# jacketsj/expANN

Hardware: AMD Instinct MI355X
Metric: queries/sec at recall@10=1.0 (exact brute force), 1Mxd128 fp32, k=10 (higher is better)
Workload: dtype f32; 1 GPU; brute_force_engine L2 N=1000000 d=128 fp32, 10000 batched queries, k=10 (BASELINE configs[1]); n=1000000, d=128, m=10000, k=10, metric=l2, launch=one process, one GPU, devices_visible=1, comm_ranks=0

## Files before the change

expann_amd/csrc/expann_hip.hip:

```cpp
#include "../../include/expann_hip.h"

#include <hip/hip_runtime.h>

#include <algorithm>
#include <cmath>
#include <cstdio>
#include <cstdlib>
#include <cstring>
#include <memory>
#include <mutex>
#include <string>
#include <vector>

#include "host_common.hpp"
#include "scan_f32.hpp"
#include "scan_gemm_bf16.hpp"
#include "scan_gemm_f16.hpp"
#include "scan_gemm_f16k.hpp"
#include "scan_gemm_f16x.hpp"
#include "scan_gemm_f16y.hpp"
#include "scan_gemm_f16kx.hpp"
#include "scan_gemm_f16kl.hpp"
#include "scan_direct_f16.hpp"
#include "scan_gemm_i8.hpp"
// ... 608 lines not shown
#define GEMM_I8(D, MODE, MN) {D, MODE, scan_gemm_i8_kernel<D, MODE>, row_self_i8_kernel<D, MODE>, \
	query_theta_i8_kernel<D, MODE>, "scan_gemm_i8<" #D "," MN ">"}
const GemmI8Variant kGemmI8[] = {
    GEMM_I8(128, kU8L2, "U8L2"), GEMM_I8(128, kI8L2, "I8L2"), GEMM_I8(128, kI8IP, "I8IP"),
    GEMM_I8(256, kU8L2, "U8L2"), GEMM_I8(256, kI8L2, "I8L2"), GEMM_I8(256, kI8IP, "I8IP"),
    GEMM_I8(768, kU8L2, "U8L2"), GEMM_I8(768, kI8L2, "I8L2"), GEMM_I8(768, kI8IP, "I8IP")};
#undef GEMM_I8

const GemmI8Variant* pick_gemm_i8(const expann_index* h, size_t m) {
	if (h->opt_scan_kernel == 1 || h->dtype == EXPANN_DTYPE_F32)
		return nullptr;
	if (h->opt_scan_kernel == 0 && (m < 96 || h->n < 4096))
		return nullptr;
	for (const auto& v : kGemmI8)
		if (v.d == h->dim && v.mode == h->int_mode)
			return &v;
	return nullptr;
}

int ensure_bias_i8(expann_index* h, const GemmI8Variant* gv, hipStream_t st) {
	if (h->d_bias_i || h->int_mode == kI8IP)
		return EXPANN_OK;
	HIP_TRY(h, hipMalloc(&h->d_bias_i, sizeof(int) * h->n));
	const uint32_t blocks = (uint32_t)((h->n + kRowsPerGroup - 1) / kRowsPerGroup);
	hipLaunchKernelGGL(gv->self, dim3(blocks), dim3(kBlock), 0, st, (const void*)h->d_base,
	                   (uint32_t)h->n, h->d_bias_i);
	HIP_TRY(h, hipGetLastError());
	return EXPANN_OK;
}

uint32_t select_longest_list(double expect, uint32_t spec_j) {
	return spec_j ? (uint32_t)(expect * (1.0 + 4.5 / std::sqrt((double)spec_j))) : 2u * (uint32_t)expect;
}
void launch_select_wave(SelectParams& sel, size_t m, uint32_t cap, hipStream_t st, uint32_t longest) {
	sel.wave_done = 0;
	hipLaunchKernelGGL((select_wave_kernel<8, 4>), dim3((uint32_t)((m + 3) / 4)), dim3(256), 0, st, sel,
	                   (uint32_t)m);
	sel.wave_done = 512;
	if (longest <= 512)
		return;
	if (cap > 512) {
		hipLaunchKernelGGL((select_wave_kernel<16, 2>), dim3((uint32_t)((m + 1) / 2)), dim3(128), 0, st, sel, (uint32_t)m);
		sel.wave_done = 1024;
	}
	if (cap > 1024 && longest > 1024) {
		hipLaunchKernelGGL((select_wave_kernel<32, 1>), dim3((uint32_t)m), dim3(64), 0, st, sel, (uint32_t)m);
		sel.wave_done = 2048;
	}
}

int ensure_hit_logs(expann_index* h, uint32_t grid, int waves, size_t m, uint32_t cap, uint32_t n_chunks,
                    uint32_t n_qtiles, uint32_t xcd_map, hipStream_t st, uint4** log, uint32_t** log_cnt,
                    uint32_t* log_cap_out) {
	const uint32_t n_logs = grid * (uint32_t)waves;
	const uint32_t log_cap = std::max<uint32_t>(
	    4096, pow2ceil((uint32_t)std::min<size_t>(4 * ((m * (size_t)cap + n_logs - 1) / n_logs), 1u << 20)));
	const size_t need = (size_t)n_logs * log_cap * 16;
	if (need > h->log_bytes || n_logs > h->log_cnt_n) {
		HIP_TRY(h, hipStreamSynchronize(st));
		h->d_log.reset();
		h->d_log_cnt.reset();
		h->log_bytes = h->log_cnt_n = 0;
		HIP_TRY(h, hipMalloc(&h->d_log, need));
		HIP_TRY(h, hipMalloc(&h->d_log_cnt, sizeof(uint32_t) * n_logs));
		h->log_bytes = need;
		h->log_cnt_n = n_logs;
	}
	*log = h->d_log.as<uint4>();
	*log_cnt = h->d_log_cnt;
	*log_cap_out = log_cap;
	h->pending_scatter.n_logs = n_logs;
	h->pending_scatter.log_cap = log_cap;
	h->pending_scatter.cap = cap;
	h->pending_scatter.n_chunks = n_chunks;
	h->pending_scatter.n_qtiles = n_qtiles;
	h->pending_scatter.xcd_map = xcd_map;
	h->pending_scatter.m = (uint32_t)m;
	h->pending_scatter.theta = nullptr;
	h->pending_scatter.key_mul = 0.0f;
	h->pending_scatter.i_mode = 0;
	return EXPANN_OK;
}

void launch_gather_logs(expann_index* h, hipStream_t st) {
	if (!h->pending_scatter.n_logs)
		return;
	const auto ps = h->pending_scatter;
	h->pending_scatter.n_logs = 0;
	const uint32_t want = std::max<uint32_t>(1, (1024 + ps.n_qtiles * 4 - 1) / (ps.n_qtiles * 4));
	const uint32_t cpb = std::max<uint32_t>(1, (ps.n_chunks + want - 1) / want);
	const uint32_t n_groups = (ps.n_chunks + cpb - 1) / cpb;
	GatherLogParams gp{h->d_log.as<const uint4>(), h->d_log_cnt.as<const uint32_t>(), ps.log_cap, ps.n_chunks,
	                   ps.n_qtiles, ps.xcd_map, ps.m, n_groups, cpb, h->d_cnt, h->d_cand, ps.cap, ps.theta, ps.key_mul,
	                   ps.i_thp, ps.i_bias, ps.i_qself, ps.i_mode, ps.i_rw};
	hipLaunchKernelGGL(gather_logs_kernel, dim3(ps.n_qtiles * 4 * n_groups), dim3(kBlock), 0, st, gp);
}

bool defer_flags(expann_index* h, hipStream_t st, int attempt) {
	if (!h->opt_async || h->host_call || attempt != 0 || h->strict_u8 || h->async_pending >= kAsyncRing)
		return false;
	if (hipMemcpyAsync(h->h_flag_ring + 8 * h->async_pending, h->d_overflow,
	                   sizeof(uint32_t) * 4 + sizeof(unsigned long long), hipMemcpyDeviceToHost, st) != hipSuccess)
		return false;
	h->h_flag_ring[8 * h->async_pending + 6] = 0;
	h->h_flag_ring[8 * h->async_pending + 7] = h->dtype == EXPANN_DTYPE_U8 ? 1u : 0u;
	h->async_pending++;
	h->async_stream = st;
	h->prof.deferred_searches++;
	return true;
}

uint32_t pick_row_chunks(uint32_t n_tiles, uint32_t n_qtiles, uint32_t slots, double overhead, uint32_t min_tiles,
                         uint32_t g_limit, long tol_pct, uint32_t* xcd) {
	const uint32_t gmax = std::max<uint32_t>(1, n_tiles / min_tiles);
	uint32_t chunks = 1, g8 = 0;
	double best = 1e300, best8 = 1e300;
	for (uint32_t g = 1; g <= std::min<uint32_t>(gmax, g_limit); ++g) {
		const uint32_t steps = (n_tiles + g - 1) / g;
		const uint64_t rounds = ((uint64_t)g * n_qtiles + slots - 1) / slots;
		const double cost = (double)rounds * (steps + overhead);
		if (cost < best * 0.999) {
			best = cost;
			chunks = g;
		}
		if (xcd && g % 8 == 0 && cost < best8 * 0.999 && (n_tiles + steps - 1) / steps == g) {
			best8 = cost;
			g8 = g;
		}
// ... 355 lines not shown
		fp.cand_cnt = h->d_cnt;
		fp.cand = h->d_cand;
		fp.cap = cap;
		const GemmI8qVariant* gs = gq;
		const uint32_t scan_slots = gs->scan_w ? (uint32_t)gs->wg_per_cu_w * (uint32_t)cus : wg_slots;
		uint32_t fchunks = pick_row_chunks(nt, nqt, scan_slots, 4.0, 8, 2048, h->opt_xcd_tolerance,
		                                   (h->opt_debug & 1024) ? nullptr : &fp.xcd_map);
		fp.tiles_per_block = (nt + fchunks - 1) / fchunks;
		fchunks = (nt + fp.tiles_per_block - 1) / fp.tiles_per_block;
		GemmI8wParams wp{};
		if (gs->scan_w) {
			wp.q = fp;
			rc = ensure_hit_logs(h, fchunks * nqt, 4, m, cap, fchunks, nqt, fp.xcd_map, st, &wp.log, &wp.log_cnt,
			                     &wp.log_cap);
			if (rc != EXPANN_OK)
				return rc;
			wp.lost = h->d_overflow;
			h->pending_scatter.i_thp = fp.thp;
			h->pending_scatter.i_bias = fp.bias;
			h->pending_scatter.i_qself = fp.qself;
			h->pending_scatter.i_mode = fp.bias ? 1 : 2;
		}
		const bool timed = h->profiling && h->ev_used < kEventPairs;
		if (timed)
			HIP_TRY(h, hipEventRecord(h->ev[h->ev_used][0], st));
		if (gs->scan_w)
			hipLaunchKernelGGL(gs->scan_w, dim3(fchunks * nqt), dim3((uint32_t)gs->threads_w), gs->lds_w, st, wp);
		else
			hipLaunchKernelGGL(gs->scan, dim3(fchunks * nqt), dim3((uint32_t)gs->threads), gs->lds, st, fp);
		if (timed) {
			HIP_TRY(h, hipEventRecord(h->ev[h->ev_used][1], st));
			h->ev_used++;
		}
		launch_gather_logs(h, st);
		if (timed || !h->profiling) {
			h->prof.scan_launches++;
			h->prof.scan_rows += h->n;
			h->prof.scan_query_tiles += nqt;
			h->prof.query_tile = kF16TQ;
			h->prof.levels = 2;
			std::snprintf(h->prof.scan_kernel, sizeof(h->prof.scan_kernel), "%s", gs->name);
		}
		HIP_TRY(h, hipGetLastError());
		mark("scan");
		SelectParams sel{};
		sel.cand = h->d_cand;
		sel.cand_cnt = h->d_cnt;
		sel.cap = cap;
		sel.k = (uint32_t)k;
		sel.id_offset = h->id_offset;
		sel.out_ids = d_ids;
		sel.out_dists = d_dists;
		sel.dim = (uint32_t)h->dim;
		sel.overflow = h->d_overflow;
		if (h->profiling)
			hipLaunchKernelGGL(sum_u32_kernel, dim3(1), dim3(1024), 0, st, sel.cand_cnt, (uint32_t)m,
			                   h->d_total);
		launch_select_wave(sel, m, cap, st, select_longest_list(1.2 * (double)k * sample_frac_for(h, k), 0));
		mark("select_wave");
		hipLaunchKernelGGL(select_topk_kernel, dim3((uint32_t)m), dim3(kBlock), sizeof(uint64_t) * cap + 16,
		                   st, sel);
		HIP_TRY(h, hipGetLastError());
		if (defer_flags(h, st, attempt)) {
			h->h_flag_ring[8 * (h->async_pending - 1) + 6] = 0;
			return EXPANN_OK;
		}
		HIP_TRY(h, hipMemcpyAsync(h->h_flags, h->d_overflow, sizeof(uint32_t) * 4 + sizeof(unsigned long long),
		                          hipMemcpyDeviceToHost, st));
		HIP_TRY(h, hipStreamSynchronize(st));
		unsigned long long tot;
		std::memcpy(&tot, h->h_flags + 4, sizeof(tot));
		h->prof.candidates = tot;
		if (h->strict_u8 && (h->h_flags[1] != 0 || h->h_flags[3] != 0))
			return kStrictReject;
		if (h->dtype == EXPANN_DTYPE_U8 && h->h_flags[1] != 0)
			return h->fail(EXPANN_ERR_UNSUPPORTED,
			               std::to_string(h->h_flags[1]) +
			                   " query values outside [0,255]: the uint8 metric "
			                   "(dist2_compressed) is only defined for 8-bit valued queries");
		if (h->h_flags[0] == 0)
			return EXPANN_OK;
		h->prof.retries++;
		if (cap >= kMaxCap || attempt >= 2)
			return kRetryGeneric;
		cap = std::min(cap * 4, kMaxCap);
	}
}

int search_pass(expann_index* h, const void* d_queries, size_t m, size_t k, uint64_t* d_ids,
                float* d_dists, hipStream_t st);
}
extern "C" int expann_create(int dim, int dtype, int metric, int device, expann_index** out);
extern "C" int expann_set_base_device(expann_index* h, const void* d_rows, size_t n, uint64_t id_offset);
extern "C" int expann_set_profiling(expann_index* h, int enable);
// ... 718 lines not shown
		gp.bias = h->d_bias_i;
		gp.n_rows = (uint32_t)h->n;
		const uint32_t n_tiles = (uint32_t)((h->n + tb - 1) / tb);
		gp.n_tiles_sel = last ? n_tiles
		                      : std::min(n_tiles, (L.n_groups_sel * kRowsPerGroup + tb - 1) / tb);
		gp.tile_stride = std::max<uint32_t>(1, n_tiles / gp.n_tiles_sel);
		gp.n_qtiles = (uint32_t)((m + kGemmI8TQ - 1) / kGemmI8TQ);
		gp.queries = d_queries;
		gp.theta = h->d_theta.as<const int>();
		gp.qself = h->d_qself;
		gp.m = (uint32_t)m;
		gp.cand_cnt = h->d_cnt;
		gp.cand = h->d_cand;
		gp.cap = cap;
		uint32_t gchunks = pick_row_chunks(gp.n_tiles_sel, gp.n_qtiles, (uint32_t)cus, 2.0, 4, 4096, 0, nullptr);
		gp.tiles_per_block = (gp.n_tiles_sel + gchunks - 1) / gchunks;
		gchunks = (gp.n_tiles_sel + gp.tiles_per_block - 1) / gp.tiles_per_block;
		if (timed)
			HIP_TRY(h, hipEventRecord(h->ev[h->ev_used][0], st));
		hipLaunchKernelGGL(gvi->scan, dim3(gchunks * gp.n_qtiles), dim3(kGemmThreads),
		                   2 * tb * h->dim, st, gp);
		passes = gp.n_qtiles;
		kname = gvi->name;
		qt_used = kGemmI8TQ;
	} else {
		if (timed)
			HIP_TRY(h, hipEventRecord(h->ev[h->ev_used][0], st));
		hipLaunchKernelGGL(sv->fn, dim3(n_chunks * n_qtiles), dim3(kBlock), 0, st, sp);
	}
	if (timed) {
		HIP_TRY(h, hipEventRecord(h->ev[h->ev_used][1], st));
		h->ev_used++;
	}
	launch_gather_logs(h, st);
	if (last && (timed || !h->profiling)) {
		h->prof.scan_launches++;
		h->prof.scan_rows += h->n;
		h->prof.scan_query_tiles += passes;
		h->prof.query_tile = qt_used;
		h->prof.levels = (uint32_t)(levels.size() - li_start + (li_start ? 1 : 0));
		std::snprintf(h->prof.scan_kernel, sizeof(h->prof.scan_kernel), "%s", kname);
	}
	HIP_TRY(h, hipGetLastError());

	SelectParams sel{};
	sel.cand = h->d_cand;
	sel.cand_cnt = first ? nullptr : h->d_cnt;
	sel.fixed_count = (first && L.classmin_blocks) ? n_chunks * 16 : L.n_groups_sel * kRowsPerGroup;
	sel.cap = cap;
	sel.k = (uint32_t)k;
	sel.id_offset = h->id_offset;
	sel.out_ids = last ? d_ids : nullptr;
	sel.out_dists = last ? d_dists : nullptr;
	sel.tau_out = last ? nullptr : h->d_tau[li & 1];
	sel.tau_prev = first ? nullptr : h->d_tau[(li + 1) & 1];
	sel.tau_row_out = last ? nullptr : h->d_tau_row[li & 1];
	sel.tau_row_prev = first ? nullptr : h->d_tau_row[(li + 1) & 1];
	sel.rerank_base = use_gemm ? (const float*)h->d_base : nullptr;
	sel.rerank_queries = use_gemm ? (const float*)d_queries : nullptr;
	sel.dim = (uint32_t)h->dim;
	sel.metric_ip = ip ? 1u : 0u;
	const float pr = ip ? 1.0f : 2.0f;
	sel.prune_eps = use_gemm ? (gvf ? pr * gemm_f16_filter_eps(h->dim)
	                                : (gvb ? gemm_bf16_filter_eps(h->dim) : gemm_filter_eps(h->dim)))
	                         : 0.0f;
	sel.prune_abs = (use_gemm && gvf)
	                    ? pr * std::ldexp(1.0f, -24) / h->f16_scale * std::sqrt((float)h->dim)
	                    : 0.0f;
	sel.bn_max = h->d_bnmax ? h->d_bnmax + (gvf ? 2 : (gvb ? 1 : 0)) : nullptr;
	sel.qnrm = (use_gemm && gvf) ? h->d_qnrm : nullptr;
	if (use_i8f) {
		sel.prune_eps = 0.0f;
		sel.prune_abs = 0.0f;
		sel.row_w = h->d_rw_i8f;
		sel.q_w = h->d_i8f_q + 2 * h->i8f_q_m;
	}
	sel.overflow = h->d_overflow;
	if (last && spec_j) {
		const RedoWs ws(redo_slots, h->dim, cap);
		sel.spec_tau = h->d_tau_s;
		sel.redo_word = h->d_overflow + 3;
		sel.redo_list = reinterpret_cast<uint32_t*>(h->d_redo.as<unsigned char>() + ws.list);
		sel.redo_cap = redo_slots;
	}
	if (last && sel.cand_cnt && (h->profiling || use_i8f))
		hipLaunchKernelGGL(sum_u32_kernel, dim3(1), dim3(1024), 0, st, sel.cand_cnt, (uint32_t)m,
		                   h->d_total);
	if (m <= 64) {
		sel.wave0_short = 1;
	} else if (sel.rerank_base && sel.cand_cnt) {
		const uint32_t sj = last ? spec_j : 0u;
		const double expect = (use_i8f ? kI8fListRatio : 1.0) * 1.2 * (sj ? (double)sj : (double)k) * sample_frac_for(h, k);
		launch_select_wave(sel, m, cap, st, select_longest_list(expect, sj));
	}
	hipLaunchKernelGGL(select_topk_kernel, dim3((uint32_t)m), dim3(kBlock),
	                   sizeof(uint64_t) * cap + 16, st, sel);
	HIP_TRY(h, hipGetLastError());
	if (last && spec_j)
		return run_redo(use_i8f);
	return EXPANN_OK;
}

int SearchPass::run_redo(bool use_i8f) {
	const RedoWs ws(redo_slots, h->dim, cap);
	unsigned char* const b = h->d_redo.as<unsigned char>();
	uint32_t* const word = h->d_overflow + 3;
	const uint32_t R = redo_slots;
	RedoCompactParams cp{};
	cp.word = word;
	cp.list = reinterpret_cast<const uint32_t*>(b + ws.list);
	cp.n_slots = R;
	cp.row_bytes = (uint32_t)h->dim * 2;
	cp.q16 = h->d_q_split;
	cp.rq16 = b + ws.q16;
	cp.qnrm = h->d_qnrm;
	cp.r_qnrm = reinterpret_cast<float*>(b + ws.qnrm);
	cp.tau = h->d_tau[levels.size() & 1];
	cp.qscale = (ip && h->opt_ip_rescale) ? h->d_qscale.as<const float>() : nullptr;
	cp.eps = gemm_f16_filter_eps(h->dim);
	cp.abs_coef = std::ldexp(1.0f, -24) / h->f16_scale * std::sqrt((float)h->dim);
	cp.mul = 0.5f * h->f16_scale * h->f16_scale;
	cp.ip = ip ? 1 : 0;
	cp.r_theta = reinterpret_cast<float*>(b + ws.theta);
	cp.r_cnt = reinterpret_cast<uint32_t*>(b + ws.cnt);
	if (use_i8f) {
		cp.q8 = h->d_q8f;
		cp.rq8 = b + ws.q8;
		cp.i8_aq = h->d_i8f_q;
		cp.i8_wq_in = h->d_i8f_q + h->i8f_q_m;
// ... 76 lines not shown
		fp.live_q = word;
		hipLaunchKernelGGL(gvf->scan_redo, dim3(chunks * nqt), dim3((uint32_t)gvf->threads), gvf->lds, st, fp);
		gp.theta = cp.r_theta;
		gp.key_mul = fp.two_inv_s2;
	}
	const uint32_t want = std::max<uint32_t>(1, (1024 + nqt * 4 - 1) / (nqt * 4));
	gp.chunks_per_block = std::max<uint32_t>(1, (chunks + want - 1) / want);
	gp.n_groups = (chunks + gp.chunks_per_block - 1) / gp.chunks_per_block;
	hipLaunchKernelGGL(gather_logs_kernel, dim3(nqt * 4 * gp.n_groups), dim3(kBlock), 0, st, gp);

	SelectParams sel{};
	sel.cand = gp.cand;
	sel.cand_cnt = gp.cand_cnt;
	sel.cap = cap;
	sel.k = (uint32_t)k;
	sel.id_offset = h->id_offset;
	sel.out_ids = d_ids;
	sel.out_dists = d_dists;
	sel.rerank_base = (const float*)h->d_base;
	sel.rerank_queries = (const float*)d_queries;
	sel.dim = (uint32_t)h->dim;
	sel.metric_ip = ip ? 1u : 0u;
	const float pr = ip ? 1.0f : 2.0f;
	sel.bn_max = h->d_bnmax + 2;
	sel.qnrm = cp.r_qnrm;
	if (use_i8f) {
		sel.row_w = h->d_rw_i8f;
		sel.q_w = cp.r_wq;
	} else {
		sel.prune_eps = pr * gemm_f16_filter_eps(h->dim);
		sel.prune_abs = pr * std::ldexp(1.0f, -24) / h->f16_scale * std::sqrt((float)h->dim);
	}
	sel.overflow = word;
	sel.wave0_short = 1;
	sel.slot_map = cp.list;
	sel.live_slots = word;
	hipLaunchKernelGGL(select_topk_kernel, dim3(R), dim3(kBlock), sizeof(uint64_t) * cap + 16, st, sel);
	HIP_TRY(h, hipGetLastError());
	return EXPANN_OK;
}

int SearchPass::check(int attempt, Next* next) {
	*next = kDone;
	if (defer_flags(h, st, attempt)) {
		float sc = gvf ? h->f16_scale : 0.0f;
		std::memcpy(&h->h_flag_ring[8 * (h->async_pending - 1) + 6], &sc, sizeof(float));
		if (i8f_ran && h->opt_i8_filter == 1)
			h->h_flag_ring[8 * (h->async_pending - 1) + 7] =
			    0x80000000u | (uint32_t)std::min<uint64_t>(i8f_cand_limit(h, m, k, spec_j), 0x3FFFFFFFu);
		if (spec_j)
			h->h_flag_ring[8 * (h->async_pending - 1) + 7] |= 0x40000000u;
		return EXPANN_OK;
	}
	HIP_TRY(h, hipMemcpyAsync(h->h_flags, h->d_overflow, sizeof(uint32_t) * 4 + sizeof(unsigned long long),
	                          hipMemcpyDeviceToHost, st));
	HIP_TRY(h, hipStreamSynchronize(st));
	unsigned long long tot;
	std::memcpy(&tot, h->h_flags + 4, sizeof(tot));
	h->prof.candidates = tot;
	if (i8f_ran && h->opt_i8_filter == 1 && tot > i8f_cand_limit(h, m, k, spec_j))
		h->i8f_state = 2;
	if (std::getenv("EXPANN_DEBUG_LISTS")) {
		std::vector<uint32_t> cnt(m);
		HIP_TRY(h, hipMemcpy(cnt.data(), h->d_cnt, sizeof(uint32_t) * m, hipMemcpyDeviceToHost));
		std::sort(cnt.begin(), cnt.end());
		std::fprintf(stderr, "[lists] attempt %d cap %u: min %u median %u p90 %u p99 %u max %u, overflow flag %u\n", attempt, cap,
		             cnt.front(), cnt[m / 2], cnt[m * 9 / 10], cnt[m * 99 / 100], cnt.back(), h->h_flags[0]);
	}
	if (gvf) {
		float qmax;
// ... 819 lines not shown
```

expann_amd/csrc/scan_gemm_f16.hpp:

```cpp
#pragma once
#include "common.hpp"
#include "scan_gemm_bf16.hpp"
#include "scan_gemm_i8f.hpp"
#include "select.hpp"

namespace expann {

typedef _Float16 f16x8 __attribute__((ext_vector_type(8)));

__host__ __device__ inline float gemm_f16_filter_eps(int d) {
	return d <= 256 ? 1.125f * 0.0009765625f
	                : 0.0009765625f + (4.0f + 4.25f * (float)d + 256.0f) * 5.9604644775390625e-08f;
}

__global__ __launch_bounds__(kBlock) void convert_f16_kernel(const float* in, size_t n_values,
                                                             float scale, _Float16* out,
                                                             uint32_t* maxabs_bits) {
	uint32_t b = 0;
	for (size_t i = (size_t)blockIdx.x * kBlock + threadIdx.x; i < n_values;
	     i += (size_t)gridDim.x * kBlock) {
		const float v = in[i];
		out[i] = (_Float16)(v * scale);
		const uint32_t vb = __builtin_bit_cast(uint32_t, v) & 0x7fffffffu;
		b = vb > b ? vb : b;
// ... 235 lines not shown
	uint32_t cap;
	uint32_t debug;
	unsigned long long* clk;
	float* sample_out;
	uint32_t n_chunks;
	uint32_t xcd_map;
	uint32_t n_big, tiles_small;
	uint4* log;
	uint32_t* log_cnt;
	uint32_t log_cap;
	uint32_t* lost;
	uint32_t* work_ctr;
	uint32_t n_items;
	uint32_t ksteps;
	const uint32_t* live_q;
};

struct GatherLogParams {
	const uint4* log;
	const uint32_t* log_cnt;
	uint32_t log_cap, n_chunks, n_qtiles, xcd_map, m;
	uint32_t n_groups, chunks_per_block;
	uint32_t* cand_cnt;
	uint64_t* cand;
	uint32_t cap;
	const float* theta;
	float key_mul;
	const int* i_thp;
	const int* i_bias;
	const int* i_qself;
	int i_mode;
	const float* i_rw;
	const uint32_t* live_q;
};
__global__ __launch_bounds__(kBlock) void gather_logs_kernel(GatherLogParams p) {
	__shared__ uint32_t cnt[64], base[64];
	const uint32_t grp = blockIdx.x % p.n_groups, qw = blockIdx.x / p.n_groups;
	const uint32_t qtile = qw >> 2, w = qw & 3;
	const uint32_t q0 = qtile * 256 + w * 64;
	if (p.live_q && qtile * 256 >= (*p.live_q & kRedoCountMask))
		return;
	if (threadIdx.x < 64)
		cnt[threadIdx.x] = 0;
	__syncthreads();
	const uint32_t lane = threadIdx.x & 63, wv = threadIdx.x >> 6;
	const uint32_t c0 = grp * p.chunks_per_block;
	const uint32_t c1 = c0 + p.chunks_per_block < p.n_chunks ? c0 + p.chunks_per_block : p.n_chunks;
	auto log_of = [&](uint32_t c, uint32_t& n) -> const uint4* {
		const uint32_t bid = p.xcd_map ? ((c >> 3) * p.n_qtiles + qtile) * 8 + (c & 7) : c * p.n_qtiles + qtile;
		const uint32_t li = bid * 4 + w;
		n = p.log_cnt[li];
		if (n > p.log_cap)
			n = p.log_cap;
		return p.log + (size_t)li * p.log_cap;
	};
	for (uint32_t c = c0 + wv; c < c1; c += kBlock / 64) {
		uint32_t n;
		const uint4* src = log_of(c, n);
		for (uint32_t i = lane; i < n; i += 64)
			atomicAdd(&cnt[(src[i].z - q0) & 63], 1u);
	}
	__syncthreads();
	if (threadIdx.x < 64) {
		const uint32_t n = cnt[threadIdx.x];
		base[threadIdx.x] = n ? atomicAdd(&p.cand_cnt[q0 + threadIdx.x], n) : 0u;
		cnt[threadIdx.x] = 0;
	}
	__syncthreads();
	for (uint32_t c = c0 + wv; c < c1; c += kBlock / 64) {
		uint32_t n;
		const uint4* src = log_of(c, n);
		for (uint32_t i = lane; i < n; i += 64) {
			const uint4 e = src[i];
			const uint32_t ql = (e.z - q0) & 63;
			const uint32_t slot = base[ql] + atomicAdd(&cnt[ql], 1u);
			if (slot < p.cap) {
				uint64_t key;
				if (p.i_mode == 3) {
					const float kappa = (float)(p.i_bias[e.y] - (int)e.x);
					key = make_key(p.i_rw[e.y] < __builtin_inff() ? kappa : -__builtin_inff(), e.y);
				} else if (p.i_mode) {
					const int dot = (int)e.x - p.i_thp[e.z];
					const int score = p.i_mode == 1 ? p.i_bias[e.y] - 2 * dot + p.i_qself[e.z] : -dot;
					key = make_key((float)score, e.y);
				} else {
					key = make_key((__builtin_bit_cast(float, e.x) + p.theta[e.z]) * p.key_mul, e.y);
				}
				p.cand[(size_t)e.z * p.cap + slot] = key;
			}
		}
	}
}

__device__ inline float max3f(float a, float b, float c) {
	return __builtin_fmaxf(__builtin_fmaxf(a, b), c);
}

template <int N> __device__ inline void wait_vm_then_barrier() {
	asm volatile("s_waitcnt vmcnt(%0) lgkmcnt(0)\n\ts_barrier" ::"n"(N) : "memory");
// ... 240 lines not shown
```

expann_amd/csrc/select.hpp:

```cpp
#pragma once
#include "common.hpp"

namespace expann {

struct SelectParams {
	const uint64_t* cand;
	const uint32_t* cand_cnt;
	uint32_t fixed_count;
	uint32_t cap;
	uint32_t k;
	uint64_t id_offset;
	uint64_t* out_ids;
	float* out_dists;
	float* tau_out;
	const float* tau_prev;
	uint32_t* tau_row_out;
	const uint32_t* tau_row_prev;
	const float* rerank_base;
	const float* rerank_queries;
	uint32_t dim;
	uint32_t metric_ip;
	float prune_eps;
	float prune_abs;
	const float* bn_max;
	uint32_t* overflow;
	uint32_t wave_done;
	uint32_t wave0_short;
	const float* qnrm;
	const float* row_w;
	const float* q_w;
	const float* spec_tau;
	uint32_t* redo_word;
	uint32_t* redo_list;
	uint32_t redo_cap;
	const uint32_t* slot_map;
	const uint32_t* live_slots;
};
constexpr uint32_t kRedoCountMask = 0xFFFFFu;
constexpr uint32_t kRedoOverflowUnit = 1u << 20;

__device__ inline void spec_check(const SelectParams& p, uint32_t qi, bool has_kth, float s_k) {
	if (!p.spec_tau || (has_kth && s_k <= p.spec_tau[qi]))
		return;
	const uint32_t slot = atomicAdd(p.redo_word, 1u) & kRedoCountMask;
	if (slot < p.redo_cap)
		p.redo_list[slot] = qi;
}

__device__ inline float i8f_cutoff(uint32_t kth_ord, float wq) {
	if (kth_ord >= 0xFF800000u)
		return __builtin_inff();
	const float c = ordered_to_float(kth_ord) + wq;
	return c + __builtin_fabsf(c) * 0x1p-18f + 1.0f;
}
__device__ inline uint32_t i8f_upper_ord(const SelectParams& p, uint64_t key) {
	const float v = key_score(key) + p.row_w[key_idx(key)];
	return float_to_ordered(v == v ? v : __builtin_inff());
}

__global__ __launch_bounds__(1024) void sum_u32_kernel(const uint32_t* in, uint32_t n,
                                                       unsigned long long* out) {
	__shared__ unsigned long long red[16];
	unsigned long long s = 0;
	for (uint32_t i = threadIdx.x; i < n; i += 1024)
		s += in[i];
	for (int off = 32; off > 0; off >>= 1)
		s += __shfl_xor(s, off);
	if ((threadIdx.x & 63) == 0)
		red[threadIdx.x >> 6] = s;
// ... 129 lines not shown
	return lo;
}

template <int PER>
__device__ inline uint2 wave_kth_largest_sparse_u32(const uint32_t (&v)[PER], uint32_t k, uint32_t* scratch,
                                                    int lane, uint32_t j = 0) {
	uint32_t mx[1] = {v[0]};
#pragma unroll
	for (int j = 1; j < PER; ++j)
		mx[0] = v[j] > mx[0] ? v[j] : mx[0];
	const uint32_t B = wave_kth_largest_u32<1>(mx, k);
	uint32_t total = 0;
#pragma unroll
	for (int j = 0; j < PER; ++j)
		total += (uint32_t)__builtin_popcountll(__builtin_amdgcn_ballot_w64(v[j] >= B));
	if (total > 64)
		return make_uint2(wave_kth_largest_u32<PER>(v, k), j ? wave_kth_largest_u32<PER>(v, j) : 0u);
	uint32_t base = 0;
#pragma unroll
	for (int j = 0; j < PER; ++j) {
		const unsigned long long mask = __builtin_amdgcn_ballot_w64(v[j] >= B);
		if (v[j] >= B)
			scratch[base + __builtin_amdgcn_mbcnt_hi((uint32_t)(mask >> 32),
			                                         __builtin_amdgcn_mbcnt_lo((uint32_t)mask, 0u))] = v[j];
		base += (uint32_t)__builtin_popcountll(mask);
	}
	__builtin_amdgcn_fence(__ATOMIC_RELEASE, "wavefront");
	__builtin_amdgcn_wave_barrier();
	__builtin_amdgcn_fence(__ATOMIC_ACQUIRE, "wavefront");
	uint32_t w[1] = {lane < (int)total ? scratch[lane] : 0u};
	return make_uint2(wave_kth_largest_u32<1>(w, k), j ? wave_kth_largest_u32<1>(w, j) : 0u);
}

template <int PER>
__device__ inline void select_wave_body(const SelectParams& p, uint32_t qi, uint32_t c, uint64_t* list,
                                        int lane) {
	const uint64_t* src = p.cand + (size_t)qi * p.cap;
	uint64_t kk[PER];
#pragma unroll
	for (int j = 0; j < PER; ++j)
		kk[j] = lane + 64 * j < (int)c ? src[lane + 64 * j] : kSentinelKey;
	const uint32_t l = lane & 15, grp = lane >> 4;
	const uint32_t qo = p.slot_map ? p.slot_map[qi] : qi;
	const float* q = p.rerank_queries + (size_t)qo * p.dim + l;
	float cutoff = __builtin_inff();
	const bool final_scores = p.rerank_base == nullptr;
	if ((p.prune_eps > 0.0f || final_scores || p.row_w) && c > p.k) {
		float qn = 0.0f;
		if (final_scores || p.row_w) {
		} else if (p.qnrm) {
			qn = p.qnrm[qi];
		} else {
			for (uint32_t t = 0; t < p.dim / 16; ++t)
				qn = __builtin_fmaf(q[16 * t], q[16 * t], qn);
			qn = reduce16_ref_order(qn);
		}
		uint32_t sc[PER];
#pragma unroll
		for (int j = 0; j < PER; ++j)
			sc[j] = (p.row_w && kk[j] != kSentinelKey) ? i8f_upper_ord(p, kk[j]) : (uint32_t)(kk[j] >> 32);
		uint32_t kth = 0xFFFFFFFFu;
		if (p.k > 24) {
			kth = wave_kth_smallest_u32<PER>(sc, p.k);
		} else
		for (uint32_t r = 0; r < p.k; ++r) {
			uint32_t mn = sc[0];
#pragma unroll
			for (int j = 1; j < PER; ++j)
				mn = min(mn, sc[j]);
			mn = wave_min_u32(mn);
			if (mn == 0xFFFFFFFFu)
				break;
			kth = mn;
#pragma unroll
			for (int j = 0; j < PER; ++j)
				sc[j] = sc[j] == mn ? 0xFFFFFFFFu : sc[j];
		}
		if (final_scores) {
			cutoff = ordered_to_float(kth);
		} else if (p.row_w) {
			cutoff = i8f_cutoff(kth, p.q_w[qi]);
		} else {
			const float bmax = p.bn_max[0];
			cutoff = ordered_to_float(kth) + p.prune_eps * (qn + 1.5f * bmax) +
			         p.prune_abs * (__builtin_sqrtf(qn) + __builtin_sqrtf(bmax));
		}
	}
	uint32_t n_s = 0;
#pragma unroll
	for (int j = 0; j < PER; ++j) {
		const bool hit = lane + 64 * j < (int)c && key_score(kk[j]) <= cutoff;
		const unsigned long long mask = __builtin_amdgcn_ballot_w64(hit);
		const uint32_t pos = n_s + __builtin_amdgcn_mbcnt_hi((uint32_t)(mask >> 32),
		                                                      __builtin_amdgcn_mbcnt_lo((uint32_t)mask, 0u));
		if (hit)
			list[pos] = kk[j];
		n_s += (uint32_t)__builtin_popcountll(mask);
	}
	asm volatile("s_waitcnt lgkmcnt(0)" ::: "memory");
	for (uint32_t i0 = 0; p.rerank_base && i0 < n_s; i0 += 16) {
		constexpr int U = 4;
		float acc[U];
		uint32_t row[U];
		const float* r[U];
#pragma unroll
		for (int u = 0; u < U; ++u) {
			const uint32_t i = i0 + 4 * u + grp;
			row[u] = key_idx(list[i < n_s ? i : 0]);
			r[u] = p.rerank_base + (size_t)row[u] * p.dim + l;
			acc[u] = 0.0f;
		}
		const uint32_t nt = p.dim / 16;
		for (uint32_t t0 = 0; t0 < nt; t0 += 8) {
			float qv[8], rv[U][8];
#pragma unroll
			for (int t = 0; t < 8; ++t)
				qv[t] = t0 + t < nt ? q[16 * (t0 + t)] : 0.0f;
#pragma unroll
			for (int u = 0; u < U; ++u)
#pragma unroll
				for (int t = 0; t < 8; ++t)
					rv[u][t] = t0 + t < nt ? r[u][16 * (t0 + t)] : 0.0f;
#pragma unroll
			for (int u = 0; u < U; ++u)
#pragma unroll
				for (int t = 0; t < 8; ++t) {
					if (t0 + t >= nt)
						continue;
					if (p.metric_ip) {
						acc[u] = __builtin_fmaf(qv[t], rv[u][t], acc[u]);
					} else {
						const float diff = qv[t] - rv[u][t];
						acc[u] = __builtin_fmaf(diff, diff, acc[u]);
					}
				}
		}
#pragma unroll
		for (int u = 0; u < U; ++u) {
			acc[u] = reduce16_ref_order(acc[u]);
			const uint32_t i = i0 + 4 * u + grp;
			if (l == 0 && i < n_s)
				list[i] = make_key(p.metric_ip ? -acc[u] : acc[u], row[u]);
		}
	}
	asm volatile("s_waitcnt lgkmcnt(0)" ::: "memory");
	if (n_s <= 256)
		wave_emit_sorted<(PER < 4 ? PER : 4)>(p, list, n_s, qo, lane);
	else
		wave_emit_sorted<PER>(p, list, n_s, qo, lane);
}

template <int PER, int WAVES>
__global__ __launch_bounds__(64 * WAVES) void select_wave_kernel(SelectParams p, uint32_t m) {
	constexpr uint32_t kSelectWaveMax = 64 * PER;
	__shared__ uint64_t lists[WAVES][kSelectWaveMax];
	const int lane = threadIdx.x & 63;
	const int wave = __builtin_amdgcn_readfirstlane(threadIdx.x >> 6);
	const uint32_t qi = blockIdx.x * WAVES + wave;
	if (qi >= m)
		return;
	const uint32_t c = p.cand_cnt ? p.cand_cnt[qi] : p.fixed_count;
	if (c > kSelectWaveMax || c > p.cap || (c <= p.wave_done && p.wave_done != 0))
		return;
	select_wave_body<PER>(p, qi, c, lists[wave], lane);
}

__global__ __launch_bounds__(kBlock) void select_topk_kernel(SelectParams p) {
	extern __shared__ __attribute__((aligned(16))) unsigned char smem_raw[];
	uint64_t* keys = reinterpret_cast<uint64_t*>(smem_raw);
	const uint32_t qi = blockIdx.x;
	const uint32_t tid = threadIdx.x;
	if (p.live_slots && qi >= (*p.live_slots & kRedoCountMask))
		return;
	const uint32_t qo = p.slot_map ? p.slot_map[qi] : qi;
	uint32_t c = p.cand_cnt ? p.cand_cnt[qi] : p.fixed_count;
	if (p.wave_done && c <= p.wave_done && c <= p.cap)
		return;
	if (p.wave0_short && c <= 2048 && c <= p.cap && 8 * (size_t)p.cap >= 16384) {
		if (tid < 64) {
			if (c <= 512)
				select_wave_body<8>(p, qi, c, keys, (int)tid);
			else
				select_wave_body<32>(p, qi, c, keys, (int)tid);
		}
		return;
	}
	if (c > p.cap) {
		if (tid == 0)
			atomicAdd(p.overflow, p.live_slots ? kRedoOverflowUnit : 1u);
		c = p.cap;
	}
	uint32_t n2 = 2;
	while (n2 < c)
		n2 <<= 1;
	const uint64_t* src = p.cand + (size_t)qi * p.cap;
	for (uint32_t i = tid; i < n2; i += kBlock)
		keys[i] = i < c ? src[i] : kSentinelKey;
// ... 200 lines not shown
```

Baseline: 6.177 million queries/s.

## Merge short and long candidate selection into one fused select_lists kernel

Replaces the chain of select_wave launches (8/16/32-per-lane tiers) plus the per-query select_topk fallback with a single select_lists_kernel. Its tail blocks handle short lists one wave per query, and a few leading blocks sweep queries whose lists exceed 512, using a four-wave chunked prune/rescore/keep-best routine. It also folds the profiling candidate-total sum into the gather_logs kernel and adds an optional clock-stamp debug path. The aim is to cut kernel launches and the serialized long-list block selection, at the cost of more complex shared-memory bookkeeping and a fixed block count for long lists.

```diff
diff --git a/expann_amd/csrc/expann_hip.hip b/expann_amd/csrc/expann_hip.hip
--- a/expann_amd/csrc/expann_hip.hip
+++ b/expann_amd/csrc/expann_hip.hip
@@ -664,21 +664,19 @@
 uint32_t select_longest_list(double expect, uint32_t spec_j) {
 	return spec_j ? (uint32_t)(expect * (1.0 + 4.5 / std::sqrt((double)spec_j))) : 2u * (uint32_t)expect;
 }
-void launch_select_wave(SelectParams& sel, size_t m, uint32_t cap, hipStream_t st, uint32_t longest) {
+bool launch_select_lists(SelectParams& sel, size_t m, hipStream_t st, double expect, uint32_t longest) {
+	uint32_t n_long = 0;
+	if (sel.k <= kSelectLongMaxK && !sel.tau_out)
+		n_long = 1.3 * expect > (double)kSelectShortMax ? (uint32_t)m
+		                                                : std::min<uint32_t>((uint32_t)m, longest > kSelectShortMax ? 256u : 32u);
 	sel.wave_done = 0;
-	hipLaunchKernelGGL((select_wave_kernel<8, 4>), dim3((uint32_t)((m + 3) / 4)), dim3(256), 0, st, sel,
-	                   (uint32_t)m);
-	sel.wave_done = 512;
-	if (longest <= 512)
-		return;
-	if (cap > 512) {
-		hipLaunchKernelGGL((select_wave_kernel<16, 2>), dim3((uint32_t)((m + 1) / 2)), dim3(128), 0, st, sel, (uint32_t)m);
-		sel.wave_done = 1024;
-	}
-	if (cap > 1024 && longest > 1024) {
-		hipLaunchKernelGGL((select_wave_kernel<32, 1>), dim3((uint32_t)m), dim3(64), 0, st, sel, (uint32_t)m);
-		sel.wave_done = 2048;
-	}
+	const dim3 grid(n_long + (uint32_t)((m + 3) / 4));
+	if (sel.clk)
+		hipLaunchKernelGGL(select_lists_kernel<true>, grid, dim3(kBlock), 0, st, sel, (uint32_t)m, n_long);
+	else
+		hipLaunchKernelGGL(select_lists_kernel<false>, grid, dim3(kBlock), 0, st, sel, (uint32_t)m, n_long);
+	sel.wave_done = kSelectShortMax;
+	return n_long != 0;
 }
 
 int ensure_hit_logs(expann_index* h, uint32_t grid, int waves, size_t m, uint32_t cap, uint32_t n_chunks,
@@ -714,9 +712,9 @@
 	return EXPANN_OK;
 }
 
-void launch_gather_logs(expann_index* h, hipStream_t st) {
+bool launch_gather_logs(expann_index* h, hipStream_t st, unsigned long long* total = nullptr) {
 	if (!h->pending_scatter.n_logs)
-		return;
+		return false;
 	const auto ps = h->pending_scatter;
 	h->pending_scatter.n_logs = 0;
 	const uint32_t want = std::max<uint32_t>(1, (1024 + ps.n_qtiles * 4 - 1) / (ps.n_qtiles * 4));
@@ -725,7 +723,9 @@
 	GatherLogParams gp{h->d_log.as<const uint4>(), h->d_log_cnt.as<const uint32_t>(), ps.log_cap, ps.n_chunks,
 	                   ps.n_qtiles, ps.xcd_map, ps.m, n_groups, cpb, h->d_cnt, h->d_cand, ps.cap, ps.theta, ps.key_mul,
 	                   ps.i_thp, ps.i_bias, ps.i_qself, ps.i_mode, ps.i_rw};
+	gp.total = total;
 	hipLaunchKernelGGL(gather_logs_kernel, dim3(ps.n_qtiles * 4 * n_groups), dim3(kBlock), 0, st, gp);
+	return true;
 }
 
 bool defer_flags(expann_index* h, hipStream_t st, int attempt) {
@@ -1147,7 +1147,7 @@
 			HIP_TRY(h, hipEventRecord(h->ev[h->ev_used][1], st));
 			h->ev_used++;
 		}
-		launch_gather_logs(h, st);
+		const bool summed = launch_gather_logs(h, st, h->profiling ? h->d_total : nullptr);
 		if (timed || !h->profiling) {
 			h->prof.scan_launches++;
 			h->prof.scan_rows += h->n;
@@ -1168,13 +1168,15 @@
 		sel.out_dists = d_dists;
 		sel.dim = (uint32_t)h->dim;
 		sel.overflow = h->d_overflow;
-		if (h->profiling)
+		if (h->profiling && !summed)
 			hipLaunchKernelGGL(sum_u32_kernel, dim3(1), dim3(1024), 0, st, sel.cand_cnt, (uint32_t)m,
 			                   h->d_total);
-		launch_select_wave(sel, m, cap, st, select_longest_list(1.2 * (double)k * sample_frac_for(h, k), 0));
+		const double expect = 1.2 * (double)k * sample_frac_for(h, k);
+		const bool served = launch_select_lists(sel, m, st, expect, select_longest_list(expect, 0));
 		mark("select_wave");
-		hipLaunchKernelGGL(select_topk_kernel, dim3((uint32_t)m), dim3(kBlock), sizeof(uint64_t) * cap + 16,
-		                   st, sel);
+		if (!served)
+			hipLaunchKernelGGL(select_topk_kernel, dim3((uint32_t)m), dim3(kBlock), sizeof(uint64_t) * cap + 16,
+			                   st, sel);
 		HIP_TRY(h, hipGetLastError());
 		if (defer_flags(h, st, attempt)) {
 			h->h_flag_ring[8 * (h->async_pending - 1) + 6] = 0;
@@ -1959,7 +1961,8 @@
 		HIP_TRY(h, hipEventRecord(h->ev[h->ev_used][1], st));
 		h->ev_used++;
 	}
-	launch_gather_logs(h, st);
+	const bool want_total = last && !first && (h->profiling || use_i8f);
+	const bool summed = launch_gather_logs(h, st, want_total ? h->d_total : nullptr);
 	if (last && (timed || !h->profiling)) {
 		h->prof.scan_launches++;
 		h->prof.scan_rows += h->n;
@@ -2010,18 +2013,35 @@
 		sel.redo_list = reinterpret_cast<uint32_t*>(h->d_redo.as<unsigned char>() + ws.list);
 		sel.redo_cap = redo_slots;
 	}
-	if (last && sel.cand_cnt && (h->profiling || use_i8f))
+	if (want_total && !summed)
 		hipLaunchKernelGGL(sum_u32_kernel, dim3(1), dim3(1024), 0, st, sel.cand_cnt, (uint32_t)m,
 		                   h->d_total);
+	bool served = false;
 	if (m <= 64) {
 		sel.wave0_short = 1;
 	} else if (sel.rerank_base && sel.cand_cnt) {
 		const uint32_t sj = last ? spec_j : 0u;
 		const double expect = (use_i8f ? kI8fListRatio : 1.0) * 1.2 * (sj ? (double)sj : (double)k) * sample_frac_for(h, k);
-		launch_select_wave(sel, m, cap, st, select_longest_list(expect, sj));
-	}
-	hipLaunchKernelGGL(select_topk_kernel, dim3((uint32_t)m), dim3(kBlock),
-	                   sizeof(uint64_t) * cap + 16, st, sel);
+		DevBuf sclk;
+		if ((h->opt_debug & 16) && last) {
+			HIP_TRY(h, sclk.alloc(5 * 8));
+			HIP_TRY(h, hipMemsetAsync(sclk.p, 0, 5 * 8, st));
+			sel.clk = sclk.as<unsigned long long>();
+		}
+		served = launch_select_lists(sel, m, st, expect, select_longest_list(expect, sj));
+		if (sel.clk) {
+			unsigned long long c[5] = {0, 0, 0, 0, 0};
+			HIP_TRY(h, hipStreamSynchronize(st));
+			HIP_TRY(h, hipMemcpy(c, sel.clk, sizeof(c), hipMemcpyDeviceToHost));
+			const double w = c[4] ? 100.0 * (double)c[4] : 1.0;
+			std::fprintf(stderr, "select short role: %llu waves; per wave keys %.2f us, prune %.2f us, re-score %.2f us, emit %.2f us\n",
+			             c[4], c[0] / w, c[1] / w, c[2] / w, c[3] / w);
+			sel.clk = nullptr;
+		}
+	}
+	if (!served)
+		hipLaunchKernelGGL(select_topk_kernel, dim3((uint32_t)m), dim3(kBlock),
+		                   sizeof(uint64_t) * cap + 16, st, sel);
 	HIP_TRY(h, hipGetLastError());
 	if (last && spec_j)
 		return run_redo(use_i8f);
@@ -2164,10 +2184,14 @@
 		sel.prune_abs = pr * std::ldexp(1.0f, -24) / h->f16_scale * std::sqrt((float)h->dim);
 	}
 	sel.overflow = word;
-	sel.wave0_short = 1;
 	sel.slot_map = cp.list;
 	sel.live_slots = word;
-	hipLaunchKernelGGL(select_topk_kernel, dim3(R), dim3(kBlock), sizeof(uint64_t) * cap + 16, st, sel);
+	if (k <= kSelectLongMaxK) {
+		hipLaunchKernelGGL(select_long_kernel, dim3(R), dim3(kBlock), 0, st, sel);
+	} else {
+		sel.wave0_short = 1;
+		hipLaunchKernelGGL(select_topk_kernel, dim3(R), dim3(kBlock), sizeof(uint64_t) * cap + 16, st, sel);
+	}
 	HIP_TRY(h, hipGetLastError());
 	return EXPANN_OK;
 }
diff --git a/expann_amd/csrc/scan_gemm_f16.hpp b/expann_amd/csrc/scan_gemm_f16.hpp
--- a/expann_amd/csrc/scan_gemm_f16.hpp
+++ b/expann_amd/csrc/scan_gemm_f16.hpp
@@ -291,6 +291,7 @@
 	int i_mode;
 	const float* i_rw;
 	const uint32_t* live_q;
+	unsigned long long* total;
 };
 __global__ __launch_bounds__(kBlock) void gather_logs_kernel(GatherLogParams p) {
 	__shared__ uint32_t cnt[64], base[64];
@@ -324,6 +325,13 @@
 		const uint32_t n = cnt[threadIdx.x];
 		base[threadIdx.x] = n ? atomicAdd(&p.cand_cnt[q0 + threadIdx.x], n) : 0u;
 		cnt[threadIdx.x] = 0;
+		if (p.total) {
+			uint32_t s = n;
+			for (int off = 32; off > 0; off >>= 1)
+				s += __shfl_xor(s, off);
+			if (threadIdx.x == 0 && s)
+				atomicAdd(p.total, (unsigned long long)s);
+		}
 	}
 	__syncthreads();
 	for (uint32_t c = c0 + wv; c < c1; c += kBlock / 64) {
diff --git a/expann_amd/csrc/select.hpp b/expann_amd/csrc/select.hpp
--- a/expann_amd/csrc/select.hpp
+++ b/expann_amd/csrc/select.hpp
@@ -35,6 +35,7 @@
 	uint32_t redo_cap;
 	const uint32_t* slot_map;
 	const uint32_t* live_slots;
+	unsigned long long* clk;
 };
 constexpr uint32_t kRedoCountMask = 0xFFFFFu;
 constexpr uint32_t kRedoOverflowUnit = 1u << 20;
@@ -230,15 +231,73 @@
 	return make_uint2(wave_kth_largest_u32<1>(w, k), j ? wave_kth_largest_u32<1>(w, j) : 0u);
 }
 
-template <int PER>
+template <int U>
+__device__ inline void wave_rescore(const SelectParams& p, const float* q, uint64_t* list, uint32_t n_s, int lane) {
+	const uint32_t l = lane & 15, grp = lane >> 4;
+	for (uint32_t i0 = 0; p.rerank_base && i0 < n_s; i0 += 4 * U) {
+		float acc[U];
+		uint32_t row[U];
+		const float* r[U];
+#pragma unroll
+		for (int u = 0; u < U; ++u) {
+			const uint32_t i = i0 + 4 * u + grp;
+			row[u] = key_idx(list[i < n_s ? i : 0]);
+			r[u] = p.rerank_base + (size_t)row[u] * p.dim + l;
+			acc[u] = 0.0f;
+		}
+		const uint32_t nt = p.dim / 16;
+		for (uint32_t t0 = 0; t0 < nt; t0 += 8) {
+			float qv[8], rv[U][8];
+#pragma unroll
+			for (int t = 0; t < 8; ++t)
+				qv[t] = t0 + t < nt ? q[16 * (t0 + t)] : 0.0f;
+#pragma unroll
+			for (int u = 0; u < U; ++u)
+#pragma unroll
+				for (int t = 0; t < 8; ++t)
+					rv[u][t] = t0 + t < nt ? r[u][16 * (t0 + t)] : 0.0f;
+#pragma unroll
+			for (int u = 0; u < U; ++u)
+#pragma unroll
+				for (int t = 0; t < 8; ++t) {
+					if (t0 + t >= nt)
+						continue;
+					if (p.metric_ip) {
+						acc[u] = __builtin_fmaf(qv[t], rv[u][t], acc[u]);
+					} else {
+						const float diff = qv[t] - rv[u][t];
+						acc[u] = __builtin_fmaf(diff, diff, acc[u]);
+					}
+				}
+		}
+#pragma unroll
+		for (int u = 0; u < U; ++u) {
+			acc[u] = reduce16_ref_order(acc[u]);
+			const uint32_t i = i0 + 4 * u + grp;
+			if (l == 0 && i < n_s)
+				list[i] = make_key(p.metric_ip ? -acc[u] : acc[u], row[u]);
+		}
+	}
+}
+
+template <int PER, bool CLK = false>
 __device__ inline void select_wave_body(const SelectParams& p, uint32_t qi, uint32_t c, uint64_t* list,
                                         int lane) {
+	unsigned long long ts[5] = {0, 0, 0, 0, 0};
+	auto stamp = [&](int i) {
+		if (CLK) {
+			asm volatile("s_waitcnt vmcnt(0) lgkmcnt(0)" ::: "memory");
+			ts[i] = wall_clock64();
+		}
+	};
+	stamp(0);
 	const uint64_t* src = p.cand + (size_t)qi * p.cap;
 	uint64_t kk[PER];
 #pragma unroll
 	for (int j = 0; j < PER; ++j)
 		kk[j] = lane + 64 * j < (int)c ? src[lane + 64 * j] : kSentinelKey;
-	const uint32_t l = lane & 15, grp = lane >> 4;
+	stamp(1);
+	const uint32_t l = lane & 15;
 	const uint32_t qo = p.slot_map ? p.slot_map[qi] : qi;
 	const float* q = p.rerank_queries + (size_t)qo * p.dim + l;
 	float cutoff = __builtin_inff();
@@ -296,71 +355,258 @@
 		n_s += (uint32_t)__builtin_popcountll(mask);
 	}
 	asm volatile("s_waitcnt lgkmcnt(0)" ::: "memory");
-	for (uint32_t i0 = 0; p.rerank_base && i0 < n_s; i0 += 16) {
-		constexpr int U = 4;
-		float acc[U];
-		uint32_t row[U];
-		const float* r[U];
-#pragma unroll
-		for (int u = 0; u < U; ++u) {
-			const uint32_t i = i0 + 4 * u + grp;
-			row[u] = key_idx(list[i < n_s ? i : 0]);
-			r[u] = p.rerank_base + (size_t)row[u] * p.dim + l;
-			acc[u] = 0.0f;
-		}
-		const uint32_t nt = p.dim / 16;
-		for (uint32_t t0 = 0; t0 < nt; t0 += 8) {
-			float qv[8], rv[U][8];
-#pragma unroll
-			for (int t = 0; t < 8; ++t)
-				qv[t] = t0 + t < nt ? q[16 * (t0 + t)] : 0.0f;
-#pragma unroll
-			for (int u = 0; u < U; ++u)
-#pragma unroll
-				for (int t = 0; t < 8; ++t)
-					rv[u][t] = t0 + t < nt ? r[u][16 * (t0 + t)] : 0.0f;
-#pragma unroll
-			for (int u = 0; u < U; ++u)
-#pragma unroll
-				for (int t = 0; t < 8; ++t) {
-					if (t0 + t >= nt)
-						continue;
-					if (p.metric_ip) {
-						acc[u] = __builtin_fmaf(qv[t], rv[u][t], acc[u]);
-					} else {
-						const float diff = qv[t] - rv[u][t];
-						acc[u] = __builtin_fmaf(diff, diff, acc[u]);
-					}
-				}
-		}
-#pragma unroll
-		for (int u = 0; u < U; ++u) {
-			acc[u] = reduce16_ref_order(acc[u]);
-			const uint32_t i = i0 + 4 * u + grp;
-			if (l == 0 && i < n_s)
-				list[i] = make_key(p.metric_ip ? -acc[u] : acc[u], row[u]);
-		}
-	}
+	stamp(2);
+	wave_rescore<4>(p, q, list, n_s, lane);
 	asm volatile("s_waitcnt lgkmcnt(0)" ::: "memory");
+	stamp(3);
 	if (n_s <= 256)
 		wave_emit_sorted<(PER < 4 ? PER : 4)>(p, list, n_s, qo, lane);
 	else
 		wave_emit_sorted<PER>(p, list, n_s, qo, lane);
-}
-
-template <int PER, int WAVES>
-__global__ __launch_bounds__(64 * WAVES) void select_wave_kernel(SelectParams p, uint32_t m) {
-	constexpr uint32_t kSelectWaveMax = 64 * PER;
-	__shared__ uint64_t lists[WAVES][kSelectWaveMax];
+	stamp(4);
+	if (CLK && lane == 0) {
+		for (int i = 0; i < 4; ++i)
+			atomicAdd(p.clk + i, ts[i + 1] - ts[i]);
+		atomicAdd(p.clk + 4, 1ull);
+	}
+}
+
+constexpr uint32_t kSelectShortMax = 512;
+constexpr uint32_t kSelectLongMaxK = 120;
+constexpr int kLongPer = 6;
+constexpr uint32_t kLongSeg = 64 * kLongPer;
+constexpr uint32_t kLongBoundsAt = 312, kLongXchAt = 504;
+static_assert(kSelectLongMaxK + kLongSeg <= kLongXchAt && 2 * (kLongXchAt - kLongBoundsAt) >= kLongSeg &&
+                  kSelectLongMaxK <= kLongBoundsAt,
+              "a wave's 512 key slots");
+
+template <int NE> __device__ inline void wave_keep_best(uint64_t* list, uint32_t n, uint32_t k, int lane) {
+	uint64_t e[NE];
+	uint32_t r[NE];
+#pragma unroll
+	for (int j = 0; j < NE; ++j) {
+		e[j] = lane + 64 * j < (int)n ? list[lane + 64 * j] : kSentinelKey;
+		r[j] = 0;
+	}
+	for (uint32_t i = 0; i < n; ++i) {
+		const uint64_t x = list[i];
+#pragma unroll
+		for (int j = 0; j < NE; ++j)
+			r[j] += x < e[j] ? 1u : 0u;
+	}
+	asm volatile("s_waitcnt lgkmcnt(0)" ::: "memory");
+#pragma unroll
+	for (int j = 0; j < NE; ++j)
+		if (e[j] != kSentinelKey && r[j] < k)
+			list[r[j]] = e[j];
+	asm volatile("s_waitcnt lgkmcnt(0)" ::: "memory");
+}
+
+__device__ inline void select_long_body(const SelectParams& p, uint32_t qi, uint32_t c, uint64_t (*lists)[kSelectShortMax],
+                                        int lane, int wave) {
+	if (c > p.cap) {
+		if (threadIdx.x == 0)
+			atomicAdd(p.overflow, p.live_slots ? kRedoOverflowUnit : 1u);
+		c = p.cap;
+	}
+	const uint64_t* src = p.cand + (size_t)qi * p.cap;
+	const uint32_t qo = p.slot_map ? p.slot_map[qi] : qi;
+	const uint32_t k = p.k;
+	uint64_t* const list = lists[wave];
+	auto xch = [&](int w) { return reinterpret_cast<uint32_t*>(&lists[w][kLongXchAt]); };
+	auto bounds = [&](int w) { return reinterpret_cast<uint32_t*>(&lists[w][kLongBoundsAt]); };
+	const float* q = p.rerank_queries + (size_t)qo * p.dim + (lane & 15);
+	const bool final_scores = p.rerank_base == nullptr;
+	const bool cut = (p.prune_eps > 0.0f || final_scores || p.row_w) && c > k;
+	float qn = 0.0f;
+	if (cut && !final_scores && !p.row_w) {
+		if (p.qnrm) {
+			qn = p.qnrm[qi];
+		} else {
+			for (uint32_t t = 0; t < p.dim / 16; ++t)
+				qn = __builtin_fmaf(q[16 * t], q[16 * t], qn);
+			qn = reduce16_ref_order(qn);
+		}
+	}
+	uint32_t run_cut = 0xFFFFFFFFu;
+	uint32_t nb = 0;
+	for (uint32_t r0 = 0; r0 < c; r0 += 4 * kLongSeg) {
+		const uint32_t chunk = c - r0 < 4 * kLongSeg ? c - r0 : 4 * kLongSeg;
+		const uint32_t seg = (chunk + 3) / 4;
+		const uint32_t s0 = (uint32_t)wave * seg < chunk ? (uint32_t)wave * seg : chunk;
+		const uint32_t len = s0 + seg < chunk ? seg : chunk - s0;
+		uint64_t kk[kLongPer];
+#pragma unroll
+		for (int j = 0; j < kLongPer; ++j)
+			kk[j] = lane + 64 * j < (int)len ? src[r0 + s0 + lane + 64 * j] : kSentinelKey;
+		float cutoff = __builtin_inff();
+		if (cut) {
+			uint32_t sc[kLongPer];
+#pragma unroll
+			for (int j = 0; j < kLongPer; ++j)
+				sc[j] = kk[j] == kSentinelKey ? 0xFFFFFFFFu
+				                              : (p.row_w ? i8f_upper_ord(p, kk[j]) : (uint32_t)(kk[j] >> 32));
+			uint32_t kth = 0xFFFFFFFFu;
+			if (len >= k && k > 24) {
+				kth = wave_kth_smallest_u32<kLongPer>(sc, k);
+			} else if (len >= k) {
+				uint32_t t[kLongPer];
+#pragma unroll
+				for (int j = 0; j < kLongPer; ++j)
+					t[j] = sc[j];
+				for (uint32_t r = 0; r < k; ++r) {
+					uint32_t mn = t[0];
+#pragma unroll
+					for (int j = 1; j < kLongPer; ++j)
+						mn = min(mn, t[j]);
+					mn = wave_min_u32(mn);
+					if (mn == 0xFFFFFFFFu)
+						break;
+					kth = mn;
+#pragma unroll
+					for (int j = 0; j < kLongPer; ++j)
+						t[j] = t[j] == mn ? 0xFFFFFFFFu : t[j];
+				}
+			}
+			if (lane == 0)
+				xch(wave)[0] = kth;
+			__syncthreads();
+			const uint32_t cut0 = min(min(xch(0)[0], xch(1)[0]), min(xch(2)[0], xch(3)[0]));
+			const bool file_any = cut0 != 0xFFFFFFFFu || chunk >= k;
+			uint32_t n0 = 0;
+			if (file_any) {
+				uint32_t* const mine = bounds(wave);
+#pragma unroll
+				for (int j = 0; j < kLongPer; ++j) {
+					const bool hit = lane + 64 * j < (int)len && sc[j] <= cut0;
+					const unsigned long long mask = __builtin_amdgcn_ballot_w64(hit);
+					if (hit)
+						mine[n0 + __builtin_amdgcn_mbcnt_hi((uint32_t)(mask >> 32),
+						                                    __builtin_amdgcn_mbcnt_lo((uint32_t)mask, 0u))] = sc[j];
+					n0 += (uint32_t)__builtin_popcountll(mask);
+				}
+			}
+			if (lane == 0)
+				xch(wave)[1] = n0;
+			__syncthreads();
+			uint32_t round_cut = cut0;
+			const uint32_t o1 = xch(0)[1], o2 = o1 + xch(1)[1], o3 = o2 + xch(2)[1], n_all = o3 + xch(3)[1];
+			if (file_any && n_all <= 512) {
+				uint32_t v[8];
+#pragma unroll
+				for (int j = 0; j < 8; ++j) {
+					const uint32_t i = (uint32_t)lane + 64 * j;
+					const int w = (i >= o1 ? 1 : 0) + (i >= o2 ? 1 : 0) + (i >= o3 ? 1 : 0);
+					const uint32_t off = i - (w == 0 ? 0u : (w == 1 ? o1 : (w == 2 ? o2 : o3)));
+					v[j] = i < n_all ? bounds(w)[off] : 0xFFFFFFFFu;
+				}
+				round_cut = wave_kth_smallest_u32<8>(v, k);
+			}
+			__syncthreads();
+			run_cut = min(run_cut, round_cut);
+			if (run_cut != 0xFFFFFFFFu) {
+				if (final_scores) {
+					cutoff = ordered_to_float(run_cut);
+				} else if (p.row_w) {
+					cutoff = i8f_cutoff(run_cut, p.q_w[qi]);
+				} else {
+					const float bmax = p.bn_max[0];
+					cutoff = ordered_to_float(run_cut) + p.prune_eps * (qn + 1.5f * bmax) +
+					         p.prune_abs * (__builtin_sqrtf(qn) + __builtin_sqrtf(bmax));
+				}
+			}
+		}
+		uint32_t n_new = 0;
+#pragma unroll
+		for (int j = 0; j < kLongPer; ++j) {
+			const bool hit = lane + 64 * j < (int)len && key_score(kk[j]) <= cutoff;
+			const unsigned long long mask = __builtin_amdgcn_ballot_w64(hit);
+			const uint32_t pos = nb + n_new + __builtin_amdgcn_mbcnt_hi((uint32_t)(mask >> 32),
+			                                                            __builtin_amdgcn_mbcnt_lo((uint32_t)mask, 0u));
+			if (hit)
+				list[pos] = kk[j];
+			n_new += (uint32_t)__builtin_popcountll(mask);
+		}
+		asm volatile("s_waitcnt lgkmcnt(0)" ::: "memory");
+		wave_rescore<2>(p, q, list + nb, n_new, lane);
+		asm volatile("s_waitcnt lgkmcnt(0)" ::: "memory");
+		const uint32_t n = nb + n_new;
+		if (n <= 128)
+			wave_keep_best<2>(list, n, k, lane);
+		else if (n <= 256)
+			wave_keep_best<4>(list, n, k, lane);
+		else
+			wave_keep_best<8>(list, n, k, lane);
+		nb = n < k ? n : k;
+	}
+	if (lane == 0)
+		xch(wave)[2] = nb;
+	__syncthreads();
+	const uint32_t e1 = xch(0)[2], e2 = e1 + xch(1)[2], e3 = e2 + xch(2)[2], total = e3 + xch(3)[2];
+	for (uint32_t i = threadIdx.x; i < total; i += kBlock) {
+		const int w = (i >= e1 ? 1 : 0) + (i >= e2 ? 1 : 0) + (i >= e3 ? 1 : 0);
+		const uint64_t x = lists[w][i - (w == 0 ? 0u : (w == 1 ? e1 : (w == 2 ? e2 : e3)))];
+		uint32_t rank = 0;
+		for (int w2 = 0; w2 < 4; ++w2) {
+			const uint32_t n2 = xch(w2)[2];
+			for (uint32_t i2 = 0; i2 < n2; ++i2)
+				rank += lists[w2][i2] < x ? 1u : 0u;
+		}
+		if (rank >= k)
+			continue;
+		if (p.out_ids)
+			p.out_ids[(size_t)qo * k + rank] = (uint64_t)key_idx(x) + p.id_offset;
+		if (p.out_dists)
+			p.out_dists[(size_t)qo * k + rank] = key_score(x);
+		if (rank == k - 1)
+			spec_check(p, qo, true, key_score(x));
+	}
+	for (uint32_t i = total + threadIdx.x; i < k; i += kBlock) {
+		if (p.out_ids)
+			p.out_ids[(size_t)qo * k + i] = ~0ull;
+		if (p.out_dists)
+			p.out_dists[(size_t)qo * k + i] = __builtin_inff();
+	}
+	if (threadIdx.x == 0 && total < k)
+		spec_check(p, qo, false, 0.0f);
+	__syncthreads();
+}
+
+template <bool CLK>
+__global__ __launch_bounds__(kBlock) void select_lists_kernel(SelectParams p, uint32_t m, uint32_t n_long) {
+	__shared__ uint64_t lists[4][kSelectShortMax];
 	const int lane = threadIdx.x & 63;
 	const int wave = __builtin_amdgcn_readfirstlane(threadIdx.x >> 6);
-	const uint32_t qi = blockIdx.x * WAVES + wave;
-	if (qi >= m)
+	if (blockIdx.x >= n_long) {
+		const uint32_t qi = (blockIdx.x - n_long) * 4 + wave;
+		if (qi >= m)
+			return;
+		const uint32_t c = p.cand_cnt[qi];
+		if (c > kSelectShortMax || c > p.cap)
+			return;
+		select_wave_body<8, CLK>(p, qi, c, lists[wave], lane);
 		return;
-	const uint32_t c = p.cand_cnt ? p.cand_cnt[qi] : p.fixed_count;
-	if (c > kSelectWaveMax || c > p.cap || (c <= p.wave_done && p.wave_done != 0))
+	}
+	for (uint32_t q0 = blockIdx.x; q0 < m; q0 += 64 * n_long) {
+		const uint32_t mine = q0 + (uint32_t)lane * n_long;
+		const uint32_t cq = mine < m ? p.cand_cnt[mine] : 0u;
+		unsigned long long todo = __builtin_amdgcn_ballot_w64(cq > kSelectShortMax || cq > p.cap);
+		while (todo) {
+			const int b = __builtin_ctzll(todo);
+			todo &= todo - 1;
+			select_long_body(p, q0 + (uint32_t)b * n_long, (uint32_t)__builtin_amdgcn_readlane((int)cq, b), lists, lane,
+			                 wave);
+		}
+	}
+}
+
+__global__ __launch_bounds__(kBlock) void select_long_kernel(SelectParams p) {
+	__shared__ uint64_t lists[4][kSelectShortMax];
+	const uint32_t qi = blockIdx.x;
+	if (p.live_slots && qi >= (*p.live_slots & kRedoCountMask))
 		return;
-	select_wave_body<PER>(p, qi, c, lists[wave], lane);
+	select_long_body(p, qi, p.cand_cnt[qi], lists, (int)(threadIdx.x & 63),
+	                 __builtin_amdgcn_readfirstlane(threadIdx.x >> 6));
 }
 
 __global__ __launch_bounds__(kBlock) void select_topk_kernel(SelectParams p) {
diff --git a/profiles/select_phase_clocks.py b/profiles/select_phase_clocks.py
--- /dev/null
+++ b/profiles/select_phase_clocks.py
@@ -0,0 +1,28 @@
+#!/usr/bin/env python3
+import os
+import sys
+
+import torch
+
+ROOT = os.path.dirname(os.path.dirname(os.path.abspath(__file__)))
+sys.path.insert(0, ROOT)
+from expann_amd import GpuBruteForceEngine
+
+n, m, d, k = 1_000_000, 10_000, 128, 10
+dev = torch.device("cuda", 0)
+g = torch.Generator(device=dev)
+g.manual_seed(1234)
+base = torch.randn(n, d, device=dev, dtype=torch.float32, generator=g)
+g.manual_seed(4321)
+queries = torch.randn(m, d, device=dev, dtype=torch.float32, generator=g)
+eng = GpuBruteForceEngine(d, "l2")
+eng.set_base_device(base.data_ptr(), n, 0)
+ids = torch.empty(m, k, dtype=torch.int64, device=dev)
+dists = torch.empty(m, k, dtype=torch.float32, device=dev)
+s = torch.cuda.current_stream(dev)
+for dbg in (0, 0, 16, 16):
+    eng.set_option("debug", dbg)
+    eng.search_device(queries.data_ptr(), m, k, ids.data_ptr(), dists.data_ptr(), s.cuda_stream)
+    s.synchronize()
+    print("debug", dbg, "scan", eng.get_profile()["scan_kernel"], file=sys.stderr)
+eng.close()
```

New measurement: 6.487 million queries/s (median of 6 runs). +5.0%, better.
